# facebookresearch/pytorch3d

Hardware: NVIDIA H100
Metric: rasterize frames/sec (fwd+bwd) 512^2 K=8 (higher is better)
Workload: dtype f32

## Files before the change

### pytorch3d_b200/csrc/binning.cuh

```cuda
#pragma once
#include <climits>

#include "common.cuh"
#include "raster_math.cuh"

namespace b200r {

constexpr uint32_t RECT_EMPTY_X = 0x0000FFFFu;

__device__ __forceinline__ void pixel_range(float vmin, float vmax, int S, float range, int& lo, int& hi) {
  const float off = range * 0.5f, scale = (float)S / range, margin = 1e-3f + 1e-6f * (float)S;
  float a = (vmin + off) * scale - 0.5f - margin;
  float b = (vmax + off) * scale - 0.5f + margin;
  a = fminf(fmaxf(a, -1.0f), (float)S + 1.0f);
  b = fminf(fmaxf(b, -2.0f), (float)S);
  lo = max(0, (int)ceilf(a));
  hi = min(S - 1, (int)floorf(b));
}

__device__ __forceinline__ uint2 bbox_to_tile_rect(float xmin, float xmax, float ymin, float ymax, int H, int W,
                                                   float rx, float ry) {
  int ix_lo, ix_hi, iy_lo, iy_hi;
  pixel_range(xmin, xmax, W, rx, ix_lo, ix_hi);
  pixel_range(ymin, ymax, H, ry, iy_lo, iy_hi);
  if (ix_lo > ix_hi || iy_lo > iy_hi) return make_uint2(RECT_EMPTY_X, 0u);
  const uint32_t tx0 = (uint32_t)(W - 1 - ix_hi) / TILE, tx1 = (uint32_t)(W - 1 - ix_lo) / TILE;
  const uint32_t ty0 = (uint32_t)(H - 1 - iy_hi) / TILE, ty1 = (uint32_t)(H - 1 - iy_lo) / TILE;
  return make_uint2(tx0 | (tx1 << 16), ty0 | (ty1 << 16));
}

__device__ __forceinline__ bool rect_empty(uint2 r) { return (r.x & 0xFFFFu) > (r.x >> 16); }

#ifndef B200R_EXP_MEMSET_NODE
static __global__ void __launch_bounds__(256) zero_ints_kernel(int* __restrict__ p, int64_t n) {
  const int64_t i = ((int64_t)blockIdx.x * 256 + threadIdx.x) * 4;
  pdl_trigger();
  if (i + 4 <= n && (reinterpret_cast<uintptr_t>(p) & 15u) == 0)
    *reinterpret_cast<int4*>(p + i) = make_int4(0, 0, 0, 0);
  else
    for (int64_t j = i; j < n && j < i + 4; ++j) p[j] = 0;
}
#endif

template <bool AGG = true>
__device__ __forceinline__ void warp_count_rect(uint2 r, int n, int TY, int TX, int* __restrict__ tile_count,
                                                int lane) {
  const bool empty = rect_empty(r);
  const int tx0 = r.x & 0xFFFF, tx1 = r.x >> 16, ty0 = r.y & 0xFFFF, ty1 = r.y >> 16;
  if (!AGG) {
    if (empty) return;
    for (int ty = ty0; ty <= ty1; ++ty)
      for (int tx = tx0; tx <= tx1; ++tx) atomicAdd(tile_count + (n * TY + ty) * TX + tx, 1);
    return;
  }
  const int w = empty ? 1 : tx1 - tx0 + 1;
  const int ntile = empty ? 0 : w * (ty1 - ty0 + 1);
  const int rounds = (int)__reduce_max_sync(0xffffffffu, (unsigned)ntile);
  int tx = tx0, ty = ty0;
  for (int i = 0; i < rounds; ++i) {
    const bool act = i < ntile;
    const int t = act ? (n * TY + ty) * TX + tx : -1 - lane;
#ifndef B200R_EXP_AGG_MATCH
    const int tprev = __shfl_up_sync(0xffffffffu, t, 1);
    const bool cont = act && lane > 0 && t == tprev;
    const unsigned conts = __ballot_sync(0xffffffffu, cont);
    if (act && !cont) {
      const unsigned after = lane == 31 ? 0u : conts >> (lane + 1);
      atomicAdd(tile_count + t, 1 + (__ffs((int)~after) - 1));
    }
#else
    const unsigned grp = __match_any_sync(0xffffffffu, t);
    if (act && lane == __ffs(grp) - 1) atomicAdd(tile_count + t, __popc(grp));
#endif
    if (++tx > tx1) {
      tx = tx0;
      ++ty;
    }
  }
}

#ifdef B200R_EXP_ORDER4
constexpr int ORDER_BITS = 16, ORDER_CLASSES = 4;
__device__ __forceinline__ int order_class(int count, int mean) {
  return count <= 0 ? 3 : (count > 2 * mean ? 0 : (count > mean ? 1 : 2));
}
#else
constexpr int ORDER_BITS = 21, ORDER_CLASSES = 3;
__device__ __forceinline__ int order_class(int count, int mean) { return count <= 0 ? 2 : (count > mean ? 0 : 1); }
#endif
__device__ __forceinline__ unsigned long long order_key(int count, int mean) {
  return 1ull << (ORDER_BITS * order_class(count, mean));
}

static __global__ void __launch_bounds__(1024) tile_scan_kernel(int* __restrict__ counts, int* __restrict__ offsets, int n,
                                                                int* __restrict__ order) {
  __shared__ long long warp_sums[32];
  __shared__ long long carry_s;
  __shared__ unsigned long long order_sums[32];
  __shared__ unsigned long long order_total, order_carry;
  __shared__ int nonempty_s;
  const int tid = threadIdx.x, lane = tid & 31, wid = tid >> 5;
  if (tid == 0) {
    carry_s = 0;
    nonempty_s = 0;
  }
  pdl_trigger();
  pdl_wait();
  __syncthreads();
  for (int base = 0; base < n; base += 8192) {
    const int i0 = base + tid * 8;
    int v[8];
    const bool vec = i0 + 8 <= n && ((reinterpret_cast<uintptr_t>(counts) | reinterpret_cast<uintptr_t>(offsets)) & 15u) == 0;
    if (vec) {
      const int4 a = *reinterpret_cast<const int4*>(counts + i0), b = *reinterpret_cast<const int4*>(counts + i0 + 4);
      v[0] = a.x; v[1] = a.y; v[2] = a.z; v[3] = a.w;
      v[4] = b.x; v[5] = b.y; v[6] = b.z; v[7] = b.w;
    } else {
#pragma unroll
      for (int j = 0; j < 8; ++j) v[j] = i0 + j < n ? counts[i0 + j] : 0;
    }
    long long total = 0;
#pragma unroll
    for (int j = 0; j < 8; ++j) total += v[j];
    if (order != nullptr) {
      int ne = 0;
#pragma unroll
      for (int j = 0; j < 8; ++j) ne += v[j] > 0 ? 1 : 0;
      ne = __reduce_add_sync(0xffffffffu, ne);
      if (lane == 0 && ne > 0) atomicAdd(&nonempty_s, ne);
    }
    long long inc = total;
#pragma unroll
    for (int d = 1; d < 32; d <<= 1) {
      const long long t = __shfl_up_sync(0xffffffffu, inc, d);
      if (lane >= d) inc += t;
    }
    if (lane == 31) warp_sums[wid] = inc;
    __syncthreads();
    if (wid == 0) {
      long long w = warp_sums[lane];
#pragma unroll
      for (int d = 1; d < 32; d <<= 1) {
        const long long t = __shfl_up_sync(0xffffffffu, w, d);
        if (lane >= d) w += t;
      }
      warp_sums[lane] = w;
    }
    __syncthreads();
    const long long carry = carry_s;
    long long excl = carry + inc - total + (wid > 0 ? warp_sums[wid - 1] : 0);
    int o[8];
#pragma unroll
    for (int j = 0; j < 8; ++j) {
      o[j] = (int)min(excl, (long long)INT_MAX);
      excl += v[j];
    }
    if (vec) {
      const int4 a = make_int4(o[0], o[1], o[2], o[3]), b = make_int4(o[4], o[5], o[6], o[7]);
      *reinterpret_cast<int4*>(offsets + i0) = a;
      *reinterpret_cast<int4*>(offsets + i0 + 4) = b;
      *reinterpret_cast<int4*>(counts + i0) = a;
      *reinterpret_cast<int4*>(counts + i0 + 4) = b;
    } else {
#pragma unroll
      for (int j = 0; j < 8; ++j)
        if (i0 + j < n) {
          offsets[i0 + j] = o[j];
          counts[i0 + j] = o[j];
        }
    }
    __syncthreads();
    if (tid == 0) carry_s = carry + warp_sums[31];
    __syncthreads();
  }
  if (tid == 0) offsets[n] = (int)min(carry_s, (long long)INT_MAX);
  if (order == nullptr) return;
  __syncthreads();
  const long long total_pairs = carry_s;
  const int mean = (int)min(total_pairs / max(nonempty_s, 1), (long long)INT_MAX);
  unsigned long long mine = 0;
  for (int i = tid; i < n; i += 1024) mine += order_key(offsets[i + 1] - offsets[i], mean);
#pragma unroll
  for (int d = 16; d > 0; d >>= 1) mine += __shfl_xor_sync(0xffffffffu, mine, d);
  if (lane == 0) order_sums[wid] = mine;
  __syncthreads();
  if (tid == 0) {
    unsigned long long t = 0;
    for (int w = 0; w < 32; ++w) t += order_sums[w];
    order_total = t;
    order_carry = 0;
  }
  __syncthreads();
  const unsigned long long total = order_total;
  const unsigned long long fmask = (1ull << ORDER_BITS) - 1;
  long long class_base[ORDER_CLASSES];
  {
    long long at = 0;
#pragma unroll
    for (int c = 0; c < ORDER_CLASSES; ++c) {
      class_base[c] = at;
      at += (long long)((total >> (ORDER_BITS * c)) & fmask);
    }
  }
  for (int base = 0; base < n; base += 8192) {
    const int i0 = base + tid * 8;
    unsigned long long k[8], tot = 0;
#pragma unroll
    for (int j = 0; j < 8; ++j) {
      k[j] = i0 + j < n ? order_key(offsets[i0 + j + 1] - offsets[i0 + j], mean) : 0ull;
      tot += k[j];
    }
    unsigned long long inc = tot;
#pragma unroll
    for (int d = 1; d < 32; d <<= 1) {
      const unsigned long long t = __shfl_up_sync(0xffffffffu, inc, d);
      if (lane >= d) inc += t;
    }
    if (lane == 31) order_sums[wid] = inc;
    __syncthreads();
    if (wid == 0) {
      unsigned long long w = order_sums[lane];
#pragma unroll
      for (int d = 1; d < 32; d <<= 1) {
        const unsigned long long t = __shfl_up_sync(0xffffffffu, w, d);
        if (lane >= d) w += t;
      }
      order_sums[lane] = w;
    }
    __syncthreads();
    unsigned long long excl = order_carry + inc - tot + (wid > 0 ? order_sums[wid - 1] : 0ull);
#pragma unroll
    for (int j = 0; j < 8; ++j) {
      if (i0 + j < n) {
        long long pos = 0;
#pragma unroll
        for (int c = 0; c < ORDER_CLASSES; ++c)
          if (k[j] == (1ull << (ORDER_BITS * c))) pos = class_base[c] + (long long)((excl >> (ORDER_BITS * c)) & fmask);
        order[pos] = i0 + j;
      }
      excl += k[j];
    }
    __syncthreads();
    if (tid == 0) order_carry += order_sums[31];
    __syncthreads();
  }
}

template <bool AGG>
static __global__ void __launch_bounds__(256)
    tile_fill_kernel(const uint4* __restrict__ rect, int64_t E, int TY, int TX, int* __restrict__ cursor,
                     int* __restrict__ pairs, int64_t capacity) {
  const int64_t e = (int64_t)blockIdx.x * blockDim.x + threadIdx.x;
  const int lane = threadIdx.x & 31;
  pdl_trigger();
  pdl_wait();
  uint4 r4 = make_uint4(RECT_EMPTY_X, 0u, 0u, 0u);
  if (e < E) r4 = __ldg(rect + e);
  const uint2 r = make_uint2(r4.x, r4.y);
  const bool empty = rect_empty(r);
  const int n = (int)r4.z;
  const int tx0 = r.x & 0xFFFF, tx1 = r.x >> 16, ty0 = r.y & 0xFFFF, ty1 = r.y >> 16;
  if (!AGG) {
    if (empty) return;
    for (int ty = ty0; ty <= ty1; ++ty)
      for (int tx = tx0; tx <= tx1; ++tx) {
        const int pos = atomicAdd(cursor + (n * TY + ty) * TX + tx, 1);
        if (pos >= 0 && (int64_t)pos < capacity) pairs[pos] = (int)e;
      }
    return;
  }
  const int w = empty ? 1 : tx1 - tx0 + 1;
  const int ntile = empty ? 0 : w * (ty1 - ty0 + 1);
  const int rounds = (int)__reduce_max_sync(0xffffffffu, (unsigned)ntile);
  int tx = tx0, ty = ty0;
  for (int i = 0; i < rounds; ++i) {
    const bool act = i < ntile;
    const int t = act ? (n * TY + ty) * TX + tx : -1 - lane;
#ifndef B200R_EXP_AGG_MATCH
    const int tprev = __shfl_up_sync(0xffffffffu, t, 1);
    const bool cont = act && lane > 0 && t == tprev;
    const unsigned conts = __ballot_sync(0xffffffffu, cont);
    const unsigned heads = __ballot_sync(0xffffffffu, act && !cont);
    const int leader = act ? 31 - __clz((int)(heads & (0xffffffffu >> (31 - lane)))) : lane;
    int base = 0;
    if (act && !cont) {
      const unsigned after = lane == 31 ? 0u : conts >> (lane + 1);
      base = atomicAdd(cursor + t, 1 + (__ffs((int)~after) - 1));
    }
    base = __shfl_sync(0xffffffffu, base, leader);
    if (act) {
      const int pos = base + (lane - leader);
#else
    const unsigned grp = __match_any_sync(0xffffffffu, t);
    const int leader = __ffs(grp) - 1;
    int base = 0;
    if (act && lane == leader) base = atomicAdd(cursor + t, __popc(grp));
    base = __shfl_sync(0xffffffffu, base, leader);
    if (act) {
      const int pos = base + __popc(grp & ((1u << lane) - 1u));
#endif
      if (pos >= 0 && (int64_t)pos < capacity) pairs[pos] = (int)e;
    }
    if (++tx > tx1) {
      tx = tx0;
      ++ty;
    }
  }
}

#ifndef B200R_BIN_CHUNK
#define B200R_BIN_CHUNK 1024
#endif
constexpr int BIN_CHUNK = B200R_BIN_CHUNK;
constexpr int BIN_MAX_TILES = 8192;

static __global__ void __launch_bounds__(256)
    tile_fill_private_kernel(const uint4* __restrict__ rect, int64_t E, int TY, int TX, int* __restrict__ cursor,
                             int* __restrict__ pairs, int64_t capacity) {
  extern __shared__ int hist[];
  const int tid = threadIdx.x, T = TY * TX;
  const int64_t e0 = (int64_t)blockIdx.x * BIN_CHUNK;
  pdl_trigger();
  for (int t = tid; t < T; t += 256) hist[t] = 0;
  pdl_wait();
  __syncthreads();
  const int n0 = (int)__ldg(rect + e0).z;
  uint2 r[BIN_CHUNK / 256];
  int own[BIN_CHUNK / 256];
#pragma unroll
  for (int i = 0; i < BIN_CHUNK / 256; ++i) {
    const int64_t e = e0 + i * 256 + tid;
    uint4 r4 = make_uint4(RECT_EMPTY_X, 0u, 0u, 0u);
    if (e < E) r4 = __ldg(rect + e);
    r[i] = make_uint2(r4.x, r4.y);
    own[i] = (int)r4.z;
  }
#pragma unroll
  for (int i = 0; i < BIN_CHUNK / 256; ++i) {
    if (rect_empty(r[i]) || own[i] != n0) continue;
    const int tx0 = r[i].x & 0xFFFF, tx1 = r[i].x >> 16, ty0 = r[i].y & 0xFFFF, ty1 = r[i].y >> 16;
    for (int ty = ty0; ty <= ty1; ++ty)
      for (int tx = tx0; tx <= tx1; ++tx) atomicAdd(hist + ty * TX + tx, 1);
  }
  __syncthreads();
#ifdef B200R_EXP_PFILL_SERIAL
// ... 236 lines not shown
```

### pytorch3d_b200/csrc/raster_meshes.cu

```cuda
#include <cfloat>
#include <climits>

#include "binning.cuh"
#include "bulk_copy.cuh"
#include "common.cuh"
#include "raster_math.cuh"

namespace b200r {

constexpr int SETUP_FACES = 256;
#ifndef B200R_MESH_TILE_H
#define B200R_MESH_TILE_H 16
#endif
constexpr int FTW = 16, FTH = B200R_MESH_TILE_H, FTHREADS = FTW * FTH;
static_assert(FTH == 16 || FTH == 8, "16x16 or 16x8 tiles");
constexpr int CHUNK = FTHREADS;
constexpr int SMEMQ_MAX_K = 32;

__device__ __forceinline__ bool face_is_drawable(const Face& f, bool cull_backfaces) {
  const float zmax = fmaxf(fmaxf(f.z0, f.z1), f.z2), zmin = fminf(fminf(f.z0, f.z1), f.z2);
  if (!(zmax >= 0.0f)) return false;
  if ((double)zmin < kEps) return false;
  const float area = edge_fn(f.x0, f.y0, f.x1, f.y1, f.x2, f.y2);
  if (cull_backfaces && area < 0.0f) return false;
// ... 1067 lines not shown
  pdl_wait();
  const int seg_begin = p.tile_offset[t], seg_end = p.tile_offset[t + 1];
  const bool overflow = (int64_t)seg_end > p.capacity || seg_end == INT_MAX;
  const int64_t mesh_first = p.first[n];
  const int count = overflow ? (int)p.num[n] : seg_end - seg_begin;
  const bool persp = p.persp != 0, clip = p.clip != 0, cull = p.cull != 0;
  const int K = p.K;

  if (!overflow && count > 1)
    cta_sort_segment<FTHREADS>(p.pairs + seg_begin, count, reinterpret_cast<int*>(&s),
                               (int)(sizeof(FaceChunk) / sizeof(int)));

  float qz[B200R_MAX_K], qd[B200R_MAX_K];
  int qi[B200R_MAX_K];
  int qn = 0, q_max_idx = -1;
  float q_max_z = -1000.0f;

  for (int base = 0; base < count; base += CHUNK) {
    const int nc = min(CHUNK, count - base);
    __syncthreads();
    if (tid < nc) {
      const int f = overflow ? (int)(mesh_first + base + tid) : p.pairs[seg_begin + base + tid];
      stage_face(s, tid, p.face_verts, p.neighbor, f, p.sqrt_blur, cull);
    }
    __syncthreads();
    for (int g = 0; g < nc; g += 32) {
      bool touch = false;
      if (g + lane < nc) {
        const float4 bx = s.box[g + lane];
        touch = !(fx_lo > bx.y || fx_hi < bx.x || fy_lo > bx.w || fy_hi < bx.z);
      }
      unsigned m = __ballot_sync(0xffffffffu, touch);
      while (m) {
        const int j = g + __ffs(m) - 1;
        m &= m - 1;
        const float4 bx = s.box[j];
        if (!valid || px > bx.y || px < bx.x || py > bx.w || py < bx.z) continue;
        const float4 fa = s.a[j], fb = s.b[j], fc = s.c[j];
        const Face f = {fa.x, fa.y, fc.x, fa.z, fa.w, fc.y, fb.x, fb.y, fc.z};
        Hit h;
        const int nb = __float_as_int(fc.w);
        if (!eval_pixel_face<false>(px, py, f, fb.z, p.blur_radius, persp, clip, qn >= K && nb == -1, q_max_z, h))
          continue;
        const int fi = __float_as_int(fb.w);
        int at = -1;
        if (nb != -1)
          for (int i = 0; i < qn; ++i)
            if (qi[i] == nb) {
              at = i;
              break;
            }
        if (at >= 0) {
          if (fabsf(h.dist) < fabsf(qd[at])) {
            qz[at] = h.z;
            qi[at] = fi;
            qd[at] = h.dist;
            if (h.z > q_max_z) {
              q_max_z = h.z;
              q_max_idx = at;
            }
          }
        } else if (qn < K) {
          qz[qn] = h.z;
          qi[qn] = fi;
          qd[qn] = h.dist;
          if (h.z > q_max_z) {
            q_max_z = h.z;
            q_max_idx = qn;
          }
          ++qn;
        } else if (h.z < q_max_z) {
          qz[q_max_idx] = h.z;
          qi[q_max_idx] = fi;
          qd[q_max_idx] = h.dist;
          q_max_z = h.z;
          for (int i = 0; i < K; ++i)
            if (qz[i] > q_max_z) {
              q_max_z = qz[i];
              q_max_idx = i;
            }
        }
      }
    }
  }
  if (!valid) return;
  for (int i = 1; i < qn; ++i) {
    const float tz = qz[i];
    const int ti = qi[i];
    int j = i - 1;
    while (j >= 0 && key_less(tz, ti, qz[j], qi[j])) {
      qz[j + 1] = qz[j];
      qi[j + 1] = qi[j];
      --j;
    }
    qz[j + 1] = tz;
    qi[j + 1] = ti;
  }
  const int64_t o = (((int64_t)n * p.H + yo) * p.W + xo) * K;
  for (int k = 0; k < K; ++k) {
    Hit h = {-1.0f, -1.0f, -1.0f, -1.0f, -1.0f};
    long long id = -1;
    if (k < qn) {
      const float* v = p.face_verts + (int64_t)qi[k] * 9;
      const Face f = {__ldg(v + 0), __ldg(v + 1), __ldg(v + 2), __ldg(v + 3), __ldg(v + 4),
                      __ldg(v + 5), __ldg(v + 6), __ldg(v + 7), __ldg(v + 8)};
      eval_pixel_face<false>(px, py, f, bary_denominator(f), p.blur_radius, persp, clip, false, 0.0f, h);
      id = qi[k];
    }
    p.pix_to_face[o + k] = id;
    p.zbuf[o + k] = h.z;
    p.dists[o + k] = h.dist;
    p.bary[(o + k) * 3 + 0] = h.b0;
    p.bary[(o + k) * 3 + 1] = h.b1;
    p.bary[(o + k) * 3 + 2] = h.b2;
  }
}

struct BackwardParams {
  const float* face_verts;
  const int64_t* pix_to_face;
  const float* grad_zbuf;
  const float* grad_bary;
  const float* grad_dists;
  int N, H, W, K, TY, TX;
  int n0;
  int g_vec;
  int64_t F;
  float rx, ry;
  int persp, clip;
  float* grad_face_verts;
  const int64_t* faces;
  float* grad_verts;
  int64_t V;
};

__device__ __forceinline__ void edge_bwd(float px, float py, float ax, float ay, float bx, float by, float g,
                                         float2& dp, float2& da, float2& db) {
  dp = make_float2(g * (by - ay), g * (ax - bx));
  da = make_float2(g * (py - by), g * (bx - px));
  db = make_float2(g * (ay - py), g * (px - ax));
}

__device__ __forceinline__ void point_line_bwd(float px, float py, float ax, float ay, float bx, float by, float g,
                                               float2& ga, float2& gb) {
  const float bax = bx - ax, bay = by - ay;
  const float t = __saturatef((bax * (px - ax) + bay * (py - ay)) / (bax * bax + bay * bay));
  const float qx = (1.0f - t) * ax + t * bx, qy = (1.0f - t) * ay + t * by;
  const float cx = 2.0f * (qx - px), cy = 2.0f * (qy - py);
  ga = make_float2(g * (1.0f - t) * cx, g * (1.0f - t) * cy);
  gb = make_float2(g * t * cx, g * t * cy);
}

__device__ __forceinline__ void backward_one(const BackwardParams& p, float px, float py, int64_t fi, float gz,
                                             float gd, float gb0, float gb1, float gb2, bool persp, bool clip,
                                             float (&out)[9]) {
  const float* v = p.face_verts + fi * 9;
  const Face f = {__ldg(v + 0), __ldg(v + 1), __ldg(v + 2), __ldg(v + 3), __ldg(v + 4),
                  __ldg(v + 5), __ldg(v + 6), __ldg(v + 7), __ldg(v + 8)};
  const float den = bary_denominator(f);
  float w0, w1, w2;
  bary_coords(px, py, f, den, w0, w1, w2);
  float c0 = w0, c1 = w1, c2 = w2;
  if (persp) bary_persp(c0, c1, c2, f.z0, f.z1, f.z2);
  float k0 = c0, k1 = c1, k2 = c2;
  if (clip) bary_clip(k0, k1, k2);
  const bool inside = c0 > 0.0f && c1 > 0.0f && c2 > 0.0f;
  const float sgd = inside ? -gd : gd;

  float2 dv0 = make_float2(0.f, 0.f), dv1 = dv0, dv2 = dv0;
  {
    const float e01 = point_line_dist(px, py, f.x0, f.y0, f.x1, f.y1);
    const float e02 = point_line_dist(px, py, f.x0, f.y0, f.x2, f.y2);
    const float e12 = point_line_dist(px, py, f.x1, f.y1, f.x2, f.y2);
    if (e01 <= e02 && e01 <= e12)
      point_line_bwd(px, py, f.x0, f.y0, f.x1, f.y1, sgd, dv0, dv1);
    else if (e02 <= e01 && e02 <= e12)
      point_line_bwd(px, py, f.x0, f.y0, f.x2, f.y2, sgd, dv0, dv2);
    else if (e12 <= e01 && e12 <= e02)
      point_line_bwd(px, py, f.x1, f.y1, f.x2, f.y2, sgd, dv1, dv2);
  }

  float g0 = gb0 + gz * f.z0, g1 = gb1 + gz * f.z1, g2 = gb2 + gz * f.z2;
  if (clip) {
    const float m0 = fmaxf(c0, 0.0f), m1 = fmaxf(c1, 0.0f), m2 = fmaxf(c2, 0.0f);
    float sum = m0 + m1 + m2, gsc = 1.0f;
    if (sum < 1e-5f) {
      gsc = 0.0f;
      sum = 1e-5f;
    }
    const float inv = __frcp_rn(sum), inv2 = gsc * inv * inv;
    const float s0 = -m0 * inv2, s1 = -m1 * inv2, s2 = -m2 * inv2;
    const float cross = g0 * s0 + g1 * s1 + g2 * s2;
    const float n0 = c0 < 0.0f ? 0.0f : g0 * inv + cross;
    const float n1 = c1 < 0.0f ? 0.0f : g1 * inv + cross;
    const float n2 = c2 < 0.0f ? 0.0f : g2 * inv + cross;
    g0 = n0;
    g1 = n1;
    g2 = n2;
  }
  float dz0 = 0.0f, dz1 = 0.0f, dz2 = 0.0f;
  if (persp) {
    const float t0 = w0 * f.z1 * f.z2, t1 = f.z0 * w1 * f.z2, t2 = f.z0 * f.z1 * w2;
    const float dn = fmaxf(t0 + t1 + t2, 1e-8f);
    const float rdn = __frcp_rn(dn);
    const float gdn = (-t0 * g0 - t1 * g1 - t2 * g2) * rdn * rdn;
    const float h0 = gdn + g0 * rdn, h1 = gdn + g1 * rdn, h2 = gdn + g2 * rdn;
    g0 = h0 * f.z1 * f.z2;
    g1 = h1 * f.z0 * f.z2;
    g2 = h2 * f.z0 * f.z1;
    dz0 = h1 * w1 * f.z2 + h2 * w2 * f.z1;
    dz1 = h0 * w0 * f.z2 + h2 * w2 * f.z0;
    dz2 = h0 * w0 * f.z1 + h1 * w1 * f.z0;
  }
  float2 bv0 = make_float2(0.f, 0.f), bv1 = bv0, bv2 = bv0;
  {
    const float rden = __frcp_rn(den);
    const float e0 = edge_fn(px, py, f.x1, f.y1, f.x2, f.y2);
    const float e1 = edge_fn(px, py, f.x2, f.y2, f.x0, f.y0);
    const float e2 = edge_fn(px, py, f.x0, f.y0, f.x1, f.y1);
    float2 dp, da, db, ap, aa, ab;
    const float garea = -(g0 * e0 + g1 * e1 + g2 * e2) * rden * rden;
    edge_bwd(f.x2, f.y2, f.x0, f.y0, f.x1, f.y1, garea, ap, aa, ab);
    bv2.x += ap.x; bv2.y += ap.y;
    bv0.x += aa.x; bv0.y += aa.y;
    bv1.x += ab.x; bv1.y += ab.y;
    edge_bwd(px, py, f.x1, f.y1, f.x2, f.y2, g0 * rden, dp, da, db);
    bv1.x += da.x; bv1.y += da.y;
    bv2.x += db.x; bv2.y += db.y;
    edge_bwd(px, py, f.x2, f.y2, f.x0, f.y0, g1 * rden, dp, da, db);
    bv2.x += da.x; bv2.y += da.y;
    bv0.x += db.x; bv0.y += db.y;
    edge_bwd(px, py, f.x0, f.y0, f.x1, f.y1, g2 * rden, dp, da, db);
    bv0.x += da.x; bv0.y += da.y;
    bv1.x += db.x; bv1.y += db.y;
  }
  out[0] = bv0.x + dv0.x;
  out[1] = bv0.y + dv0.y;
  out[2] = gz * k0 + dz0;
  out[3] = bv1.x + dv1.x;
  out[4] = bv1.y + dv1.y;
  out[5] = gz * k1 + dz1;
  out[6] = bv2.x + dv2.x;
  out[7] = bv2.y + dv2.y;
  out[8] = gz * k2 + dz2;
}

__device__ __forceinline__ void red_add_v2(float* addr, float a, float b) {
  asm volatile("red.global.add.v2.f32 [%0], {%1, %2};" ::"l"(addr), "f"(a), "f"(b) : "memory");
}
__device__ __forceinline__ void warp_scatter(const BackwardParams& p, int face, float (&g)[9], int lane) {
  const unsigned grp = __match_any_sync(0xffffffffu, face);
  const unsigned above = lane == 31 ? 0u : grp & (0xffffffffu << (lane + 1));
  int next = (face >= 0 && above != 0u) ? __ffs((int)above) - 1 : -1;
  while (__any_sync(0xffffffffu, next >= 0)) {
    const int src = next >= 0 ? next : lane;
#pragma unroll
    for (int i = 0; i < 9; ++i) {
      const float v = __shfl_sync(0xffffffffu, g[i], src);
      if (next >= 0) g[i] += v;
    }
    const int nn = __shfl_sync(0xffffffffu, next, src);
    next = next >= 0 ? nn : -1;
  }
  if (face >= 0 && lane == __ffs((int)grp) - 1) {
    if (p.faces != nullptr) {
      const int64_t* fc = p.faces + (int64_t)face * 3;
#pragma unroll
      for (int j = 0; j < 3; ++j) {
        const int64_t vi = __ldg(fc + j);
        if (vi < 0 || vi >= p.V) continue;
        float* o = p.grad_verts + vi * 3;
#ifndef B200R_EXP_BWD_SCALAR_RED
        if (p.g_vec) {
          const bool odd = (vi & 1) != 0;
          const float s1 = odd ? g[3 * j] : g[3 * j + 2];
          const float a = odd ? g[3 * j + 1] : g[3 * j], b = odd ? g[3 * j + 2] : g[3 * j + 1];
          if (s1 != 0.0f) atomicAdd(o + (odd ? 0 : 2), s1);
          if (a != 0.0f || b != 0.0f) red_add_v2(o + (odd ? 1 : 0), a, b);
          continue;
        }
#endif
#pragma unroll
        for (int c = 0; c < 3; ++c)
          if (g[3 * j + c] != 0.0f) atomicAdd(o + c, g[3 * j + c]);
      }
    } else {
      float* o = p.grad_face_verts + (int64_t)face * 9;
#ifndef B200R_EXP_BWD_SCALAR_RED
      if (p.g_vec) {
        const int odd = face & 1;
        atomicAdd(o + (odd ? 0 : 8), odd ? g[0] : g[8]);
#pragma unroll
        for (int j = 0; j < 4; ++j)
          red_add_v2(o + 2 * j + odd, odd ? g[2 * j + 1] : g[2 * j], odd ? g[2 * j + 2] : g[2 * j + 1]);
        return;
      }
#endif
#pragma unroll
      for (int i = 0; i < 9; ++i) atomicAdd(o + i, g[i]);
    }
  }
}

#ifndef B200R_BWD_PF_CTAS
#define B200R_BWD_PF_CTAS 3
#endif
#ifndef B200R_BWD_CTAS
#define B200R_BWD_CTAS 4
#endif
template <int GV, bool PF>
__global__ void __launch_bounds__(TILE_THREADS, PF ? B200R_BWD_PF_CTAS : B200R_BWD_CTAS) mesh_backward_kernel(const BackwardParams p) {
  const int lane = threadIdx.x & 31;
  const int tile_x = blockIdx.x, tile_y = blockIdx.y, n = p.n0 + blockIdx.z;
  int xo, yo;
  thread_pixel(tile_x, tile_y, xo, yo);
  const bool in_image = xo < p.W && yo < p.H;
  const float px = pix_to_ndc(p.W - 1 - xo, p.W, p.rx);
  const float py = pix_to_ndc(p.H - 1 - yo, p.H, p.ry);
  const int K = p.K;
  const int64_t o = in_image ? (((int64_t)n * p.H + yo) * p.W + xo) * K : 0;
  const bool persp = p.persp != 0, clip = p.clip != 0;
  constexpr int G = GV > 0 ? GV : 1;
  static_assert(!PF || GV == 8, "the prefetching variant is the K % 8 == 0 kernel");

  for (int k0 = 0; k0 < K; k0 += G) {
    int fk[G];
    if (GV > 0) {
#pragma unroll
      for (int k = 0; k < G; k += 2) {
        longlong2 v = make_longlong2(-1, -1);
        if (in_image) v = __ldg(reinterpret_cast<const longlong2*>(p.pix_to_face + o + k0 + k));
        fk[k] = (int)v.x;
        fk[k + 1] = (int)v.y;
      }
    } else {
      fk[0] = in_image ? (int)p.pix_to_face[o + k0] : -1;
    }
    float pz[PF ? 4 : 1], pd[PF ? 4 : 1], pb[PF ? 12 : 1];
    if (PF) {
      float4 vz = make_float4(0.f, 0.f, 0.f, 0.f), vd = vz, b0 = vz, b1 = vz, b2 = vz;
      if (fk[0] >= 0) {
        vz = __ldg(reinterpret_cast<const float4*>(p.grad_zbuf + o + k0));
        vd = __ldg(reinterpret_cast<const float4*>(p.grad_dists + o + k0));
        const float4* gb = reinterpret_cast<const float4*>(p.grad_bary + (o + k0) * 3);
        b0 = __ldg(gb + 0);
        b1 = __ldg(gb + 1);
        b2 = __ldg(gb + 2);
      }
      pz[0] = vz.x; pz[1] = vz.y; pz[2] = vz.z; pz[3] = vz.w;
      pd[0] = vd.x; pd[1] = vd.y; pd[2] = vd.z; pd[3] = vd.w;
      pb[0] = b0.x; pb[1] = b0.y; pb[2] = b0.z; pb[3] = b0.w;
      pb[4] = b1.x; pb[5] = b1.y; pb[6] = b1.z; pb[7] = b1.w;
      pb[8] = b2.x; pb[9] = b2.y; pb[10] = b2.z; pb[11] = b2.w;
    }
#pragma unroll 1
    for (int j = 0; j < G; ++j) {
      const int face = fk[0];
#pragma unroll
      for (int u = 0; u + 1 < G; ++u) fk[u] = fk[u + 1];
      float gz = 0.f, gd = 0.f, gb0 = 0.f, gb1 = 0.f, gb2 = 0.f;
      if (PF) {
        gz = pz[0]; gd = pd[0]; gb0 = pb[0]; gb1 = pb[1]; gb2 = pb[2];
#pragma unroll
        for (int u = 0; u < 3; ++u) {
          pz[u] = pz[u + 1];
          pd[u] = pd[u + 1];
        }
#pragma unroll
        for (int u = 0; u < 9; ++u) pb[u] = pb[u + 3];
      }
      if (!__any_sync(0xffffffffu, face >= 0)) continue;
      float g[9] = {0.f, 0.f, 0.f, 0.f, 0.f, 0.f, 0.f, 0.f, 0.f};
      if (face >= 0) {
        const int64_t i = o + k0 + j;
        if (!PF || j >= 4) {
          gz = __ldg(p.grad_zbuf + i);
          gd = __ldg(p.grad_dists + i);
          gb0 = __ldg(p.grad_bary + i * 3);
          gb1 = __ldg(p.grad_bary + i * 3 + 1);
          gb2 = __ldg(p.grad_bary + i * 3 + 2);
        }
        backward_one(p, px, py, face, gz, gd, gb0, gb1, gb2, persp, clip, g);
      }
      warp_scatter(p, face, g, lane);
    }
  }
}

}

__global__ void __launch_bounds__(256) mesh_gather_kernel(const float* __restrict__ verts, int64_t V,
                                                          const int64_t* __restrict__ faces, int64_t F,
                                                          float* __restrict__ face_verts_out) {
  const int64_t e = (int64_t)blockIdx.x * blockDim.x + threadIdx.x;
  if (e >= F * 3) return;
  const int64_t vi = __ldg(faces + e);
  const bool ok = vi >= 0 && vi < V;
#pragma unroll
  for (int c = 0; c < 3; ++c) face_verts_out[e * 3 + c] = ok ? __ldg(verts + vi * 3 + c) : __int_as_float(0x7fc00000);
}

using namespace b200r;

extern "C" size_t b200r_rasterize_meshes_workspace_bytes(int64_t F, int32_t N, int32_t H, int32_t W,
                                                         int64_t pair_capacity) {
  if (F < 0 || N < 0 || H < 0 || W < 0) return 0;
  return carve_workspace(nullptr, F, N, H, W, pair_capacity, FTH, FTW).bytes +
         FACE_RECORD_BYTES * (size_t)(F > 0 ? F : 1);
}

static int forward_impl(const float* face_verts, const float* verts, int64_t V, const int64_t* faces,
                        float* face_verts_out, int64_t F, const int64_t* first, const int64_t* num,
                        const int64_t* neighbor, int32_t N, int32_t H, int32_t W, float blur_radius, int32_t K,
                        int32_t perspective_correct, int32_t clip_barycentric_coords, int32_t cull_backfaces,
                        int64_t* pix_to_face, float* zbuf, float* bary, float* dists, void* workspace,
                        size_t workspace_bytes, int64_t pair_capacity, void* stream_) {
  cudaStream_t stream = static_cast<cudaStream_t>(stream_);
  if (K > B200R_MAX_K) return fail(B200R_ERR_INVALID_ARGUMENT, "Must have points_per_pixel <= 150");
  if (F < 0 || N < 0 || H < 0 || W < 0 || K < 0) return fail(B200R_ERR_INVALID_ARGUMENT, "negative size");
  if (F > INT_MAX) return fail(B200R_ERR_INVALID_ARGUMENT, "more than 2^31-1 packed faces are not supported");
  if ((int64_t)N * H * W * K == 0) return B200R_OK;
  const int TY = div_up(H, FTH), TX = div_up(W, FTW);
  if (TY > 0xFFFE || TX > 0xFFFE) return fail(B200R_ERR_INVALID_ARGUMENT, "image too large");
  const int64_t ntiles = (int64_t)N * TY * TX;
  if (ntiles > INT_MAX) return fail(B200R_ERR_INVALID_ARGUMENT, "too many tiles");
  BinWorkspace ws = carve_workspace(workspace, F, N, H, W, pair_capacity, FTH, FTW);
  const size_t nrec = (size_t)(F > 0 ? F : 1);
  if (workspace == nullptr || workspace_bytes < ws.bytes + FACE_RECORD_BYTES * nrec)
    return fail(B200R_ERR_WORKSPACE, "workspace too small for rasterize_meshes_forward");
  float4* rec = reinterpret_cast<float4*>(static_cast<char*>(workspace) + ws.bytes);

  const float rx = ndc_range(W, H), ry = ndc_range(H, W);
  const float sqrt_blur = sqrtf(blur_radius);

  const bool prof = profiling_enabled();
  if (prof) phase_timer().record(0, stream);
#ifndef B200R_EXP_MEMSET_NODE
  zero_ints_kernel<<<(unsigned)((ntiles + 1023) / 1024), 256, 0, stream>>>(ws.tile_count, ntiles);
  B200R_LAUNCHED("zero_ints_kernel");
#else
  B200R_CUDA_OK(cudaMemsetAsync(ws.tile_count, 0, sizeof(int) * (size_t)ntiles, stream));
#endif
  if (F > 0) {
    const unsigned sgrid = (unsigned)((F + SETUP_FACES - 1) / SETUP_FACES);
#ifndef B200R_EXP_MEMSET_NODE
#define B200R_SETUP_LAUNCH(KERNEL, ...) B200R_CUDA_OK(launch_chained(KERNEL, dim3(sgrid), dim3(SETUP_FACES), 0, stream, __VA_ARGS__))
#else
#define B200R_SETUP_LAUNCH(KERNEL, ...) KERNEL<<<sgrid, SETUP_FACES, 0, stream>>>(__VA_ARGS__)
#endif
    if (faces != nullptr) {
      B200R_SETUP_LAUNCH(mesh_setup_count_kernel<true>, (const float*)nullptr, verts, V, faces, face_verts_out, neighbor, F,
                         first, num, N, H, W, TY, TX, rx, ry, sqrt_blur, cull_backfaces, ws.rect, ws.tile_count, rec);
      face_verts = face_verts_out;
    } else {
      B200R_SETUP_LAUNCH(mesh_setup_count_kernel<false>, face_verts, (const float*)nullptr, (int64_t)0,
                         (const int64_t*)nullptr, (float*)nullptr, neighbor, F, first, num, N, H, W, TY, TX, rx, ry,
                         sqrt_blur, cull_backfaces, ws.rect, ws.tile_count, rec);
    }
#undef B200R_SETUP_LAUNCH
    B200R_LAUNCHED("mesh_setup_count_kernel");
  }
#ifdef B200R_EXP_NOTILEORDER
  int* const tile_order = nullptr;
#else
  int* const tile_order = (blur_radius > 0.0f && ntiles < (1ll << ORDER_BITS)) ? ws.tile_order : nullptr;
#endif
  B200R_CUDA_OK(launch_chained(tile_scan_kernel, dim3(1), dim3(1024), 0, stream, ws.tile_count, ws.tile_offset,
                               (int)ntiles, tile_order));
  B200R_LAUNCHED("tile_scan_kernel");
  if (F > 0) {
    B200R_CUDA_OK(launch_chained(tile_fill_kernel<true>, dim3((unsigned)((F + 255) / 256)), dim3(256), 0, stream,
                                 ws.rect, F, TY, TX, ws.tile_count, ws.pairs, ws.capacity));
    B200R_LAUNCHED("tile_fill_kernel");
  }
  if (prof) phase_timer().record(1, stream);
  FineParams p;
  p.face_verts = face_verts;
  p.neighbor = neighbor;
  p.rec = rec;
  p.n0 = 0;
  p.first = first;
  p.num = num;
  p.tile_offset = ws.tile_offset;
  p.tile_order = tile_order;
  p.pairs = ws.pairs;
  p.capacity = ws.capacity;
  p.N = N; p.H = H; p.W = W; p.K = K; p.TY = TY; p.TX = TX;
  p.rx = rx; p.ry = ry; p.blur_radius = blur_radius; p.sqrt_blur = sqrt_blur;
  p.persp = perspective_correct; p.clip = clip_barycentric_coords; p.cull = cull_backfaces;
  p.smem_ints = 0;
  p.pix_to_face = pix_to_face; p.zbuf = zbuf; p.bary = bary; p.dists = dists;
  const unsigned grid = (unsigned)ntiles;
  const bool no_blur = !(blur_radius > 0.0f);
  int dev_ = 0;
  B200R_CUDA_OK(cudaGetDevice(&dev_));
#define B200R_FINE_LAUNCH(KERNEL, SMEM_MAX, SMEM)                                                         \
  do {                                                                                                   \
    static bool configured[64] = {};                                                                     \
    if (dev_ < 0 || dev_ >= 64 || !configured[dev_]) {                                                   \
      B200R_CUDA_OK(cudaFuncSetAttribute(KERNEL, cudaFuncAttributeMaxDynamicSharedMemorySize, (int)(SMEM_MAX))); \
      if (dev_ >= 0 && dev_ < 64) configured[dev_] = true;                                               \
    }                                                                                                    \
    p.smem_ints = (int)((SMEM) / sizeof(int));                                                           \
    for (p.n0 = 0; p.n0 < N; p.n0 += 65535) {                                                            \
      const dim3 grid3((unsigned)TX, (unsigned)TY, (unsigned)min(N - p.n0, 65535));                      \
      B200R_CUDA_OK(launch_chained(KERNEL, grid3, dim3(FTHREADS), (SMEM), stream, p));                   \
    }                                                                                                    \
  } while (0)
#define B200R_FINE(KM)                                                                                    \
  do {                                                                                                   \
    constexpr size_t smem_ = sizeof(FineStage) + sizeof(float4) * KM * FTHREADS;                         \
    if (neighbor && no_blur)                                                                             \
      B200R_FINE_LAUNCH((mesh_fine_kernel<KM, true, true>), smem_, smem_);                               \
    else if (neighbor)                                                                                   \
      B200R_FINE_LAUNCH((mesh_fine_kernel<KM, true, false>), smem_, smem_);                              \
    else if (no_blur)                                                                                    \
      B200R_FINE_LAUNCH((mesh_fine_kernel<KM, false, true>), smem_, smem_);                              \
    else                                                                                                 \
      B200R_FINE_LAUNCH((mesh_fine_kernel<KM, false, false>), smem_, smem_);                             \
  } while (0)
  if (K <= 1)
    B200R_FINE(1);
  else if (K <= 2)
    B200R_FINE(2);
  else if (K <= 4)
    B200R_FINE(4);
  else if (K <= 8)
    B200R_FINE(8);
  else if (K <= SMEMQ_MAX_K) {
    const size_t smem_max_nb = sizeof(FineStage) + (size_t)SMEMQ_MAX_K * FTHREADS * 12;
    const size_t smem_max = sizeof(FineStage) + (size_t)SMEMQ_MAX_K * FTHREADS * 8;
    const size_t smem_nb = sizeof(FineStage) + (size_t)K * FTHREADS * 12;
    const size_t smem = sizeof(FineStage) + (size_t)K * FTHREADS * 8;
    if (neighbor && no_blur)
      B200R_FINE_LAUNCH((mesh_fine_smemq_kernel<true, true>), smem_max_nb, smem_nb);
    else if (neighbor)
      B200R_FINE_LAUNCH((mesh_fine_smemq_kernel<true, false>), smem_max_nb, smem_nb);
    else if (no_blur)
      B200R_FINE_LAUNCH((mesh_fine_smemq_kernel<false, true>), smem_max, smem);
    else
      B200R_FINE_LAUNCH((mesh_fine_smemq_kernel<false, false>), smem_max, smem);
  } else
    B200R_CUDA_OK(launch_chained(mesh_fine_bigk_kernel, dim3(grid), dim3(FTHREADS), 0, stream, p));
#undef B200R_FINE
#undef B200R_FINE_LAUNCH
  B200R_LAUNCHED("mesh_fine_kernel");
  if (prof) {
    phase_timer().record(2, stream);
    phase_timer().have_fwd = true;
  }
  return B200R_OK;
}

extern "C" int b200r_rasterize_meshes_forward(const float* face_verts, int64_t F, const int64_t* first,
                                              const int64_t* num, const int64_t* neighbor, int32_t N, int32_t H,
                                              int32_t W, float blur_radius, int32_t K, int32_t bin_size,
                                              int32_t max_faces_per_bin, int32_t perspective_correct,
                                              int32_t clip_barycentric_coords, int32_t cull_backfaces,
                                              int64_t* pix_to_face, float* zbuf, float* bary, float* dists,
                                              void* workspace, size_t workspace_bytes, int64_t pair_capacity,
                                              void* stream_) {
  (void)bin_size;
  (void)max_faces_per_bin;
  return forward_impl(face_verts, nullptr, 0, nullptr, nullptr, F, first, num, neighbor, N, H, W, blur_radius, K,
                      perspective_correct, clip_barycentric_coords, cull_backfaces, pix_to_face, zbuf, bary, dists,
                      workspace, workspace_bytes, pair_capacity, stream_);
}

extern "C" int b200r_rasterize_meshes_forward_indexed(const float* verts, int64_t V, const int64_t* faces, int64_t F,
                                                      const int64_t* first, const int64_t* num,
                                                      const int64_t* neighbor, int32_t N, int32_t H, int32_t W,
                                                      float blur_radius, int32_t K, int32_t perspective_correct,
                                                      int32_t clip_barycentric_coords, int32_t cull_backfaces,
                                                      int64_t* pix_to_face, float* zbuf, float* bary, float* dists,
                                                      float* face_verts_out, void* workspace,
                                                      size_t workspace_bytes, int64_t pair_capacity,
                                                      void* stream_) {
  if (V < 0) return fail(B200R_ERR_INVALID_ARGUMENT, "negative size");
  if (F > 0 && (faces == nullptr || face_verts_out == nullptr || (V > 0 && verts == nullptr)))
    return fail(B200R_ERR_INVALID_ARGUMENT, "verts, faces and face_verts_out must not be null");
  if ((int64_t)N * H * W * K == 0 && F > 0) {
    cudaStream_t stream = static_cast<cudaStream_t>(stream_);
    mesh_gather_kernel<<<(unsigned)((F * 3 + 255) / 256), 256, 0, stream>>>(verts, V, faces, F, face_verts_out);
    B200R_LAUNCHED("mesh_gather_kernel");
    return B200R_OK;
  }
  return forward_impl(nullptr, verts, V, F > 0 ? faces : nullptr, face_verts_out, F, first, num, neighbor, N, H, W,
                      blur_radius, K, perspective_correct, clip_barycentric_coords, cull_backfaces, pix_to_face,
                      zbuf, bary, dists, workspace, workspace_bytes, pair_capacity, stream_);
}

static int backward_impl(const float* face_verts, int64_t F, const int64_t* pix_to_face, const float* grad_zbuf,
                         const float* grad_bary, const float* grad_dists, int32_t N, int32_t H, int32_t W, int32_t K,
                         int32_t perspective_correct, int32_t clip_barycentric_coords, float* grad_face_verts,
                         const int64_t* faces, float* grad_verts, int64_t V, void* stream_) {
  cudaStream_t stream = static_cast<cudaStream_t>(stream_);
  if (F < 0 || N < 0 || H < 0 || W < 0 || K < 0) return fail(B200R_ERR_INVALID_ARGUMENT, "negative size");
  if (F == 0) return B200R_OK;
  if (faces == nullptr) B200R_CUDA_OK(cudaMemsetAsync(grad_face_verts, 0, sizeof(float) * 9 * (size_t)F, stream));
  if ((int64_t)N * H * W * K == 0) return B200R_OK;
  const int TY = div_up(H, TILE), TX = div_up(W, TILE);
  BackwardParams p;
  p.face_verts = face_verts; p.pix_to_face = pix_to_face;
  p.grad_zbuf = grad_zbuf; p.grad_bary = grad_bary; p.grad_dists = grad_dists;
  p.N = N; p.H = H; p.W = W; p.K = K; p.TY = TY; p.TX = TX;
  p.F = F;
  p.g_vec = (reinterpret_cast<uintptr_t>(faces != nullptr ? grad_verts : grad_face_verts) & 7u) == 0 ? 1 : 0;
  p.rx = ndc_range(W, H); p.ry = ndc_range(H, W);
  p.persp = perspective_correct; p.clip = clip_barycentric_coords;
  p.grad_face_verts = grad_face_verts;
  p.faces = faces;
  p.grad_verts = grad_verts;
  p.V = V;
  const bool prof = profiling_enabled();
  if (prof) phase_timer().record(3, stream);
  for (p.n0 = 0; p.n0 < N; p.n0 += 65535) {
    const dim3 bgrid((unsigned)TX, (unsigned)TY, (unsigned)min(N - p.n0, 65535));
    const bool aligned = ((reinterpret_cast<uintptr_t>(grad_zbuf) | reinterpret_cast<uintptr_t>(grad_bary) |
                           reinterpret_cast<uintptr_t>(grad_dists)) & 15u) == 0;
#ifdef B200R_EXP_BWDPF
    const bool prefetch = aligned;
#else
    const bool prefetch = false && aligned;
#endif
    if ((K & 7) == 0 && prefetch)
      mesh_backward_kernel<8, true><<<bgrid, TILE_THREADS, 0, stream>>>(p);
    else if ((K & 7) == 0)
      mesh_backward_kernel<8, false><<<bgrid, TILE_THREADS, 0, stream>>>(p);
    else if ((K & 3) == 0)
      mesh_backward_kernel<4, false><<<bgrid, TILE_THREADS, 0, stream>>>(p);
    else
      mesh_backward_kernel<0, false><<<bgrid, TILE_THREADS, 0, stream>>>(p);
  }
  B200R_LAUNCHED("mesh_backward_kernel");
  if (prof) {
    phase_timer().record(4, stream);
    phase_timer().have_bwd = true;
  }
  return B200R_OK;
}

extern "C" int b200r_rasterize_meshes_backward(const float* face_verts, int64_t F, const int64_t* pix_to_face,
                                               const float* grad_zbuf, const float* grad_bary,
                                               const float* grad_dists, int32_t N, int32_t H, int32_t W, int32_t K,
                                               int32_t perspective_correct, int32_t clip_barycentric_coords,
                                               float* grad_face_verts, void* stream_) {
  return backward_impl(face_verts, F, pix_to_face, grad_zbuf, grad_bary, grad_dists, N, H, W, K, perspective_correct,
                       clip_barycentric_coords, grad_face_verts, nullptr, nullptr, 0, stream_);
}

extern "C" int b200r_rasterize_meshes_backward_indexed(const float* face_verts, const int64_t* faces, int64_t F,
                                                       int64_t V, const int64_t* pix_to_face,
                                                       const float* grad_zbuf, const float* grad_bary,
                                                       const float* grad_dists, int32_t N, int32_t H, int32_t W,
                                                       int32_t K, int32_t perspective_correct,
                                                       int32_t clip_barycentric_coords, float* grad_verts,
                                                       float* grad_face_verts_scratch, void* stream_) {
  cudaStream_t stream = static_cast<cudaStream_t>(stream_);
  if (F < 0 || V < 0) return fail(B200R_ERR_INVALID_ARGUMENT, "negative size");
  if (V > 0) B200R_CUDA_OK(cudaMemsetAsync(grad_verts, 0, sizeof(float) * 3 * (size_t)V, stream));
  if (F == 0 || V == 0) return B200R_OK;
  (void)grad_face_verts_scratch;
  return backward_impl(face_verts, F, pix_to_face, grad_zbuf, grad_bary, grad_dists, N, H, W, K, perspective_correct,
                       clip_barycentric_coords, nullptr, faces, grad_verts, V, stream_);
}
```

Before: 18500.

## Stage backward gradients via cp.async and chain backward launches with PDL

Replaces the disabled register-prefetch backward variant with a shared-memory staged variant. For K multiple of 8 and K>8 it copies grad_zbuf, grad_dists, grad_bary and the face ids into shared memory with cp.async, only up to the last valid face, and lets the warp stop at the largest per-warp window. The gradient-zeroing memsets become a zero_ints_kernel, and all backward kernels launch through launch_chained with pdl_wait, so launch setup and prologue loads can overlap the previous kernel. The staged path needs dynamic shared memory, which may reduce occupancy, and it does not run for K=8 since it requires K>8.

```diff
diff --git a/pytorch3d_b200/csrc/binning.cuh b/pytorch3d_b200/csrc/binning.cuh
--- a/pytorch3d_b200/csrc/binning.cuh
+++ b/pytorch3d_b200/csrc/binning.cuh
@@ -31,16 +31,15 @@
 
 __device__ __forceinline__ bool rect_empty(uint2 r) { return (r.x & 0xFFFFu) > (r.x >> 16); }
 
-#ifndef B200R_EXP_MEMSET_NODE
 static __global__ void __launch_bounds__(256) zero_ints_kernel(int* __restrict__ p, int64_t n) {
   const int64_t i = ((int64_t)blockIdx.x * 256 + threadIdx.x) * 4;
+  pdl_wait();
   pdl_trigger();
   if (i + 4 <= n && (reinterpret_cast<uintptr_t>(p) & 15u) == 0)
     *reinterpret_cast<int4*>(p + i) = make_int4(0, 0, 0, 0);
   else
     for (int64_t j = i; j < n && j < i + 4; ++j) p[j] = 0;
 }
-#endif
 
 template <bool AGG = true>
 __device__ __forceinline__ void warp_count_rect(uint2 r, int n, int TY, int TX, int* __restrict__ tile_count,
diff --git a/pytorch3d_b200/csrc/raster_meshes.cu b/pytorch3d_b200/csrc/raster_meshes.cu
--- a/pytorch3d_b200/csrc/raster_meshes.cu
+++ b/pytorch3d_b200/csrc/raster_meshes.cu
@@ -1393,14 +1393,20 @@
   }
 }
 
-#ifndef B200R_BWD_PF_CTAS
-#define B200R_BWD_PF_CTAS 3
-#endif
+__device__ __forceinline__ void cp_async16(void* smem, const void* gmem) {
+  asm volatile("cp.async.cg.shared.global [%0], [%1], 16;" ::"r"(smem_u32(smem)), "l"(gmem) : "memory");
+}
+__device__ __forceinline__ void cp_async_commit_wait_all() {
+  asm volatile("cp.async.commit_group;\n\tcp.async.wait_group 0;" ::: "memory");
+}
+
+constexpr int bwd_stage_pieces(int gv) { return gv * 6 / 4; }
 #ifndef B200R_BWD_CTAS
 #define B200R_BWD_CTAS 4
 #endif
-template <int GV, bool PF>
-__global__ void __launch_bounds__(TILE_THREADS, PF ? B200R_BWD_PF_CTAS : B200R_BWD_CTAS) mesh_backward_kernel(const BackwardParams p) {
+template <int GV, bool STAGED>
+__global__ void __launch_bounds__(TILE_THREADS, B200R_BWD_CTAS) mesh_backward_kernel(const BackwardParams p) {
+  extern __shared__ __align__(16) unsigned char smem_raw[];
   const int lane = threadIdx.x & 31;
   const int tile_x = blockIdx.x, tile_y = blockIdx.y, n = p.n0 + blockIdx.z;
   int xo, yo;
@@ -1412,7 +1418,10 @@
   const int64_t o = in_image ? (((int64_t)n * p.H + yo) * p.W + xo) * K : 0;
   const bool persp = p.persp != 0, clip = p.clip != 0;
   constexpr int G = GV > 0 ? GV : 1;
-  static_assert(!PF || GV == 8, "the prefetching variant is the K % 8 == 0 kernel");
+  static_assert(!STAGED || GV == 8, "the staging variant is the K % 8 == 0 kernel");
+  float* const col = reinterpret_cast<float*>(smem_raw) + threadIdx.x * 4;
+  auto piece = [&](int q) { return col + q * (4 * TILE_THREADS); };
+  auto staged = [&](int q) { return piece(q >> 2)[q & 3]; };
 
   for (int k0 = 0; k0 < K; k0 += G) {
     int fk[G];
@@ -1427,44 +1436,57 @@
     } else {
       fk[0] = in_image ? (int)p.pix_to_face[o + k0] : -1;
     }
-    float pz[PF ? 4 : 1], pd[PF ? 4 : 1], pb[PF ? 12 : 1];
-    if (PF) {
-      float4 vz = make_float4(0.f, 0.f, 0.f, 0.f), vd = vz, b0 = vz, b1 = vz, b2 = vz;
-      if (fk[0] >= 0) {
-        vz = __ldg(reinterpret_cast<const float4*>(p.grad_zbuf + o + k0));
-        vd = __ldg(reinterpret_cast<const float4*>(p.grad_dists + o + k0));
-        const float4* gb = reinterpret_cast<const float4*>(p.grad_bary + (o + k0) * 3);
-        b0 = __ldg(gb + 0);
-        b1 = __ldg(gb + 1);
-        b2 = __ldg(gb + 2);
-      }
-      pz[0] = vz.x; pz[1] = vz.y; pz[2] = vz.z; pz[3] = vz.w;
-      pd[0] = vd.x; pd[1] = vd.y; pd[2] = vd.z; pd[3] = vd.w;
-      pb[0] = b0.x; pb[1] = b0.y; pb[2] = b0.z; pb[3] = b0.w;
-      pb[4] = b1.x; pb[5] = b1.y; pb[6] = b1.z; pb[7] = b1.w;
-      pb[8] = b2.x; pb[9] = b2.y; pb[10] = b2.z; pb[11] = b2.w;
+    int window = 0;
+    if (STAGED) {
+#pragma unroll
+      for (int k = 0; k < G; ++k) window = fk[k] >= 0 ? k + 1 : window;
+      const float* gz = p.grad_zbuf + o + k0;
+      const float* gd = p.grad_dists + o + k0;
+      const float* gb = p.grad_bary + (o + k0) * 3;
+#pragma unroll
+      for (int q = 0; q < G / 4; ++q) {
+        if (4 * q < window) {
+          cp_async16(piece(q), gz + 4 * q);
+          cp_async16(piece(G / 4 + q), gd + 4 * q);
+        }
+      }
+#pragma unroll
+      for (int q = 0; q < 3 * G / 4; ++q)
+        if (4 * q < 3 * window) cp_async16(piece(G / 2 + q), gb + 4 * q);
+#pragma unroll
+      for (int q = 0; q < G / 4; ++q)
+        if (4 * q < window)
+          *reinterpret_cast<int4*>(piece(5 * G / 4 + q)) = make_int4(fk[4 * q], fk[4 * q + 1], fk[4 * q + 2], fk[4 * q + 3]);
+    }
+    if (k0 == 0) pdl_wait();
+    int slots = G;
+    if (STAGED) {
+      slots = (int)__reduce_max_sync(0xffffffffu, (unsigned)window);
+      if (slots == 0) continue;
+      cp_async_commit_wait_all();
     }
 #pragma unroll 1
-    for (int j = 0; j < G; ++j) {
-      const int face = fk[0];
-#pragma unroll
-      for (int u = 0; u + 1 < G; ++u) fk[u] = fk[u + 1];
-      float gz = 0.f, gd = 0.f, gb0 = 0.f, gb1 = 0.f, gb2 = 0.f;
-      if (PF) {
-        gz = pz[0]; gd = pd[0]; gb0 = pb[0]; gb1 = pb[1]; gb2 = pb[2];
-#pragma unroll
-        for (int u = 0; u < 3; ++u) {
-          pz[u] = pz[u + 1];
-          pd[u] = pd[u + 1];
-        }
-#pragma unroll
-        for (int u = 0; u < 9; ++u) pb[u] = pb[u + 3];
+    for (int j = 0; j < slots; ++j) {
+      int face;
+      if (STAGED) {
+        face = j < window ? __float_as_int(staged(5 * G + j)) : -1;
+      } else {
+        face = fk[0];
+#pragma unroll
+        for (int u = 0; u + 1 < G; ++u) fk[u] = fk[u + 1];
       }
       if (!__any_sync(0xffffffffu, face >= 0)) continue;
       float g[9] = {0.f, 0.f, 0.f, 0.f, 0.f, 0.f, 0.f, 0.f, 0.f};
       if (face >= 0) {
-        const int64_t i = o + k0 + j;
-        if (!PF || j >= 4) {
+        float gz, gd, gb0, gb1, gb2;
+        if (STAGED) {
+          gz = staged(j);
+          gd = staged(G + j);
+          gb0 = staged(2 * G + 3 * j);
+          gb1 = staged(2 * G + 3 * j + 1);
+          gb2 = staged(2 * G + 3 * j + 2);
+        } else {
+          const int64_t i = o + k0 + j;
           gz = __ldg(p.grad_zbuf + i);
           gd = __ldg(p.grad_dists + i);
           gb0 = __ldg(p.grad_bary + i * 3);
@@ -1688,7 +1710,11 @@
   cudaStream_t stream = static_cast<cudaStream_t>(stream_);
   if (F < 0 || N < 0 || H < 0 || W < 0 || K < 0) return fail(B200R_ERR_INVALID_ARGUMENT, "negative size");
   if (F == 0) return B200R_OK;
-  if (faces == nullptr) B200R_CUDA_OK(cudaMemsetAsync(grad_face_verts, 0, sizeof(float) * 9 * (size_t)F, stream));
+  if (faces == nullptr) {
+    B200R_CUDA_OK(launch_chained(zero_ints_kernel, dim3((unsigned)((9 * F + 1023) / 1024)), dim3(256), 0, stream,
+                                 reinterpret_cast<int*>(grad_face_verts), 9 * F));
+    B200R_LAUNCHED("zero_ints_kernel");
+  }
   if ((int64_t)N * H * W * K == 0) return B200R_OK;
   const int TY = div_up(H, TILE), TX = div_up(W, TILE);
   BackwardParams p;
@@ -1705,23 +1731,21 @@
   p.V = V;
   const bool prof = profiling_enabled();
   if (prof) phase_timer().record(3, stream);
+  const bool staged = (K & 7) == 0 && K > 8 &&
+                      ((reinterpret_cast<uintptr_t>(grad_zbuf) | reinterpret_cast<uintptr_t>(grad_bary) |
+                        reinterpret_cast<uintptr_t>(grad_dists)) & 15u) == 0;
+  constexpr size_t stage_bytes = sizeof(float4) * bwd_stage_pieces(8) * TILE_THREADS;
   for (p.n0 = 0; p.n0 < N; p.n0 += 65535) {
     const dim3 bgrid((unsigned)TX, (unsigned)TY, (unsigned)min(N - p.n0, 65535));
-    const bool aligned = ((reinterpret_cast<uintptr_t>(grad_zbuf) | reinterpret_cast<uintptr_t>(grad_bary) |
-                           reinterpret_cast<uintptr_t>(grad_dists)) & 15u) == 0;
-#ifdef B200R_EXP_BWDPF
-    const bool prefetch = aligned;
-#else
-    const bool prefetch = false && aligned;
-#endif
-    if ((K & 7) == 0 && prefetch)
-      mesh_backward_kernel<8, true><<<bgrid, TILE_THREADS, 0, stream>>>(p);
+    const dim3 block(TILE_THREADS);
+    if (staged)
+      B200R_CUDA_OK(launch_chained(mesh_backward_kernel<8, true>, bgrid, block, stage_bytes, stream, p));
     else if ((K & 7) == 0)
-      mesh_backward_kernel<8, false><<<bgrid, TILE_THREADS, 0, stream>>>(p);
+      B200R_CUDA_OK(launch_chained(mesh_backward_kernel<8, false>, bgrid, block, 0, stream, p));
     else if ((K & 3) == 0)
-      mesh_backward_kernel<4, false><<<bgrid, TILE_THREADS, 0, stream>>>(p);
+      B200R_CUDA_OK(launch_chained(mesh_backward_kernel<4, false>, bgrid, block, 0, stream, p));
     else
-      mesh_backward_kernel<0, false><<<bgrid, TILE_THREADS, 0, stream>>>(p);
+      B200R_CUDA_OK(launch_chained(mesh_backward_kernel<0, false>, bgrid, block, 0, stream, p));
   }
   B200R_LAUNCHED("mesh_backward_kernel");
   if (prof) {
@@ -1749,7 +1773,11 @@
                                                        float* grad_face_verts_scratch, void* stream_) {
   cudaStream_t stream = static_cast<cudaStream_t>(stream_);
   if (F < 0 || V < 0) return fail(B200R_ERR_INVALID_ARGUMENT, "negative size");
-  if (V > 0) B200R_CUDA_OK(cudaMemsetAsync(grad_verts, 0, sizeof(float) * 3 * (size_t)V, stream));
+  if (V > 0) {
+    B200R_CUDA_OK(launch_chained(zero_ints_kernel, dim3((unsigned)((3 * V + 1023) / 1024)), dim3(256), 0, stream,
+                                 reinterpret_cast<int*>(grad_verts), 3 * V));
+    B200R_LAUNCHED("zero_ints_kernel");
+  }
   if (F == 0 || V == 0) return B200R_OK;
   (void)grad_face_verts_scratch;
   return backward_impl(face_verts, F, pix_to_face, grad_zbuf, grad_bary, grad_dists, N, H, W, K, perspective_correct,
```

Result: no change. 18660 (median of 6 runs) (+0.8%).
